# aquaskyline/SOAPdenovo-Trans

Hardware: AMD Instinct MI355X
Metric: pregraph k-mers hashed/sec (higher is better)
Workload: dtype u64

## Files before the change

soapdenovo-trans_amd/__init__.py:

```python
from __future__ import annotations

import ctypes
import os
import subprocess

import numpy as np

PKG_DIR = os.path.dirname(os.path.abspath(__file__))
CSRC_DIR = os.path.join(PKG_DIR, "csrc")
LIB_PATH = os.path.join(CSRC_DIR, "libsdt_gpu.so")
REPO_ROOT = os.path.dirname(PKG_DIR)

SDT_FLAG_DIRECT, SDT_FLAG_PARTITION, SDT_FLAG_TRACK_FIRST, SDT_FLAG_KEEP_READS, SDT_FLAG_CONTIG_INDEX = 1, 2, 4, 8, 16
SDT_OK, SDT_EINVAL, SDT_ENODEV, SDT_ENOMEM, SDT_EHIP, SDT_EFULL, SDT_ESTATE, SDT_ELIMIT = 0, -1, -2, -3, -4, -5, -6, -7

_c = ctypes
_ABI = [
    ("sdt_gpu_init", _c.c_int, [_c.POINTER(_c.c_void_p), _c.c_int, _c.c_int, _c.c_uint64, _c.c_uint32]),
    ("sdt_gpu_destroy", _c.c_int, [_c.c_void_p]),
    ("sdt_gpu_last_error", _c.c_char_p, []),
    ("sdt_gpu_abi_version", _c.c_int, []),
    ("sdt_gpu_reset", _c.c_int, [_c.c_void_p]),
    ("sdt_gpu_push_reads", _c.c_int, [_c.c_void_p, _c.c_void_p, _c.c_uint64, _c.c_void_p, _c.c_uint64]),
    ("sdt_gpu_push_reads_async", _c.c_int, [_c.c_void_p, _c.c_void_p, _c.c_uint64, _c.c_void_p, _c.c_uint64, _c.POINTER(_c.c_uint64)]),
# ... 888 lines not shown
        return fr[: n.value], to[: n.value], mult[: n.value], first[: n.value]

    def export_paths(self):
        n = ctypes.c_uint64()
        self._check(self.lib.sdt_gpu_export_paths(self._ctx, None, None, 0, ctypes.byref(n)))
        m = max(n.value, 1)
        keys = np.zeros((m, self.nw), dtype=np.uint64)
        words = np.zeros(m, dtype=np.uint64)
        self._check(self.lib.sdt_gpu_export_paths(self._ctx, _ptr(keys), _ptr(words), m, ctypes.byref(n)))
        return keys[: n.value], words[: n.value]

    def import_paths(self, keys, path_words, patch_keys=None, patch_info=None, num_ed: int = 0):
        keys = np.ascontiguousarray(keys, dtype=np.uint64).reshape(-1, self.nw)
        path_words = np.ascontiguousarray(path_words, dtype=np.uint64)
        assert len(keys) == len(path_words)
        pk, pi, npatch = self._patch_args(patch_keys, patch_info)
        self._check(self.lib.sdt_gpu_import_paths(self._ctx, _ptr(keys), _ptr(path_words), len(path_words), _ptr(pk), _ptr(pi), npatch,
                                                  num_ed))

    def keep_reads(self, words: np.ndarray, offsets: np.ndarray):
        words = np.ascontiguousarray(words, dtype=np.uint32)
        offsets = np.ascontiguousarray(offsets, dtype=np.uint64)
        self._check(self.lib.sdt_gpu_keep_reads(self._ctx, _ptr(words), words.size, _ptr(offsets), offsets.size - 1))

    def release_table(self):
        self._check(self.lib.sdt_gpu_release_table(self._ctx))

    def table_slots(self) -> int:
        return self.lib.sdt_gpu_table_slots(self._ctx)

    def table_info(self) -> dict:
        a = np.zeros(8, dtype=np.uint64)
        self._check(self.lib.sdt_gpu_table_info(self._ctx, a.ctypes.data))
        return {"layout": "flat", "slots": int(a[1]), "nodes": int(a[2])}

    def stream(self) -> int:
        return self.lib.sdt_gpu_stream(self._ctx) or 0

    def set_stream(self, hip_stream: int):
        self._check(self.lib.sdt_gpu_set_stream(self._ctx, ctypes.c_void_p(hip_stream)))

    def kernel_time(self, reset: bool = True):
        ms, launches, kmers = ctypes.c_double(), ctypes.c_uint64(), ctypes.c_uint64()
        self._check(self.lib.sdt_gpu_kernel_time(self._ctx, int(reset), ctypes.byref(ms), ctypes.byref(launches),
                                                 ctypes.byref(kmers)))
        return ms.value, launches.value, kmers.value

    def stage_times(self):
        ms = (ctypes.c_double * 5)()
        cnt = (ctypes.c_uint64 * 20)()
        self._check(self.lib.sdt_gpu_stage_times(self._ctx, ms, cnt))
        names = ("merges", "lds_spills", "pool_direct", "early_flushes", "chunks_l1", "chunks_l2", "batches", "batch_kmers", "cnt_ticks_setup",
                 "cnt_ticks_fill", "cnt_ticks_count", "cnt_ticks_merge", "sc_ticks_stage", "sc_ticks_minima", "sc_ticks_starts",
                 "sc_ticks_emit", "distinct_records", "records", "distinct_record_kmers", "reserved1")
        return [float(x) for x in ms], dict(zip(names, (int(x) for x in cnt)))


def new_comm_id() -> bytes:
    buf = ctypes.create_string_buffer(128)
    if load_library().sdt_gpu_comm_id(buf) != SDT_OK:
        raise SdtError(SDT_EHIP, load_library().sdt_gpu_last_error().decode())
    return buf.raw


def count_plan(off2, kpre2, first_limit, limit, max_launches=4096):
    o = np.ascontiguousarray(off2, dtype=np.uint32)
    kp = np.ascontiguousarray(kpre2, dtype=np.uint64)
    nb = len(o) - 1
    assert len(kp) == nb + 1
    cap = nb + int(o[-1]) // 1024 + 2
    items = np.zeros((cap, 4), dtype=np.uint32)
    first = np.zeros(max_launches + 2, dtype=np.uint32)
    lk = np.zeros(max_launches + 2, dtype=np.uint64)
    ni, nl = ctypes.c_uint32(), ctypes.c_uint32()
    rc = load_library().sdt_sk_plan_count_items(o.ctypes.data, kp.ctypes.data, nb, first_limit, limit, max_launches, items.ctypes.data, cap,
                                                first.ctypes.data, lk.ctypes.data, len(first), ctypes.addressof(ni), ctypes.addressof(nl))
    if rc != 0:
        raise SdtError(rc, load_library().sdt_gpu_last_error().decode())
    return items[: ni.value].copy(), first[: nl.value + 1].copy(), lk[: nl.value].copy()


def shard_cut_ranges(mat: np.ndarray, nranks: int) -> np.ndarray:
    m = np.ascontiguousarray(mat, dtype=np.uint32).reshape(nranks, 257)
    r = np.zeros(nranks + 1, dtype=np.uint32)
    rc = load_library().sdt_shard_cut_ranges(m.ctypes.data, nranks, r.ctypes.data)
    if rc != SDT_OK:
        raise SdtError(rc, load_library().sdt_gpu_last_error().decode())
    return r


def shard_plan(mat: np.ndarray, nranks: int, me: int, ranges: np.ndarray, recv_chunks: int, t: int):
    m = np.ascontiguousarray(mat, dtype=np.uint32).reshape(nranks, 257)
    rg = np.ascontiguousarray(ranges, dtype=np.uint32)
    S = ctypes.c_uint32()
    out = [np.zeros(nranks, dtype=np.uint32) for _ in range(5)]
    rc = load_library().sdt_shard_plan(m.ctypes.data, nranks, me, rg.ctypes.data, recv_chunks, t, ctypes.addressof(S),
                                       *[o.ctypes.data for o in out])
    if rc != SDT_OK:
        raise SdtError(rc, load_library().sdt_gpu_last_error().decode())
    return (S.value, *out)


def kmer_owner(key_words_msw_first, K: int, nranks: int) -> int:
    a = np.ascontiguousarray(key_words_msw_first, dtype=np.uint64)
    return load_library().sdt_kmer_owner(a.ctypes.data, K, nranks)


# ... 19 lines not shown
```

soapdenovo-trans_amd/csrc/sdt_ctx.hpp:

```cpp
#pragma once
#include <hip/hip_runtime.h>
#include <stdint.h>
#include <stdio.h>
#include <stdlib.h>
#include <string.h>
#include <stdarg.h>
#include <vector>
#include <new>
#include <thread>
#include <mutex>
#include <atomic>

#include "sdt_internal.hpp"
#include "sdt_superkmer.cuh"

using namespace sdt;
using sdti::fail;
#include "sdt_comm.cuh"
#include "sdt_shard_plan.h"
static_assert(SHARD_NB1 == SK_NB1, "the exchange plan and the pipeline agree about the level-1 buckets");

struct ArcEnt;

struct EventPair {
	hipEvent_t a, b;
	uint64_t kmers;
	int stage;
};

struct sdt_ctx {
	int device = 0;
	int K = 0;
	int nw = 1;
	uint64_t slots = 0;
	void *d_ent = nullptr;
	uint32_t *d_aux = nullptr;
	uint64_t *d_first = nullptr;
	uint64_t ord_base = 0, ord_stride = 1;
	Stats *d_stats = nullptr;
	Stats *h_stats = nullptr;
	unsigned long long *d_hist = nullptr;
	hipStream_t stream = nullptr, copy_stream = nullptr;
	bool own_stream = true;
	static constexpr int NSTAGE = 48, STAGE_AHEAD = 32;
	uint32_t *d_words[NSTAGE] = {};
	uint64_t *d_offs[NSTAGE] = {};
	uint64_t cap_words[NSTAGE] = {}, cap_offs[NSTAGE] = {};
	hipEvent_t buf_free[NSTAGE] = {}, copied[NSTAGE] = {};
	int next_buf = 0;
	struct Staged { const uint32_t *dw; uint64_t *dof; uint64_t nreads, maxlen, ord_base, ord_stride; int slot; uint64_t fixed_len; };
	std::vector<Staged> staged;
	size_t staged_head = 0;
	bool draining = false;
	uint64_t push_ord_base = 0, push_ord_stride = 1;
	uint64_t push_ticket = 0;
	uint64_t expect_kmers = 0;
	uint64_t distinct_known = 0;
	uint64_t kmers_known = 0;
	uint64_t kmers_since_sync = 0;
	uint64_t hard_since_sync = 0;
	uint64_t kmers_total_host = 0;
	uint64_t kmers_offered = 0;
	uint32_t flags = 0;
	struct SkState {
		bool ready = false;
		uint64_t cap_kmers = 0;
		bool cap_is_max = false;
		uint64_t pending_kmers = 0;
		SkPool p1 = {nullptr, nullptr, nullptr, 0}, p2 = {nullptr, nullptr, nullptr, 0};
		unsigned long long *cursors = nullptr;
		unsigned long long *blk = nullptr;
		uint32_t wgs = 0;
		uint32_t *cnt1 = nullptr, *off1 = nullptr, *fill1 = nullptr, *list1 = nullptr;
		uint32_t *cnt2 = nullptr, *off2 = nullptr, *fill2 = nullptr, *list2 = nullptr;
		unsigned long long *kmers2 = nullptr, *kpre2 = nullptr;
		SkItem *items = nullptr;
		uint32_t items_cap = 0;
		uint4 *citems = nullptr, *h_citems = nullptr;
		uint32_t citems_cap = 0;
		uint32_t *next_item = nullptr;
		uint32_t *h_off1 = nullptr, *h_off2 = nullptr;
		unsigned long long *h_kpre2 = nullptr;
		SkItem *h_items = nullptr;
		bool flushing = false;
		uint64_t st_records = 0, st_chunks1 = 0, st_chunks2 = 0, st_flushes = 0;
		uint32_t stream_flushes = 0;
		uint64_t l2_in_total = 0;
		bool exchanged = false;
	} sk;
	Comm comm;
	struct Shard {
		uint64_t *send[2] = {nullptr, nullptr}, *recv[2] = {nullptr, nullptr};
		uint32_t *send_meta[2] = {nullptr, nullptr}, *recv_meta[2] = {nullptr, nullptr};
		uint32_t *iota = nullptr;
		uint32_t send_chunks = 0, recv_chunks = 0;
		hipEvent_t ev_gather[2] = {nullptr, nullptr}, ev_xdone[2] = {nullptr, nullptr}, ev_l2[2] = {nullptr, nullptr};
		bool x_recorded[2] = {false, false}, l2_recorded[2] = {false, false};
		uint64_t round = 0;
		bool pending = false;
		int pending_slot = 0;
		uint32_t pending_items = 0;
		std::vector<SkItem> items;
		uint64_t kmers_scattered = 0;
		bool have_ranges = false;
		uint32_t ranges[65] = {0};
	} sh;
	struct KeptBatch { uint32_t *d_words; uint64_t *d_offs; uint64_t nwords, nreads, ord_base, ord_stride, maxlen; };
	std::vector<KeptBatch> kept;
	struct KeepSlab { uint8_t *p; size_t size, used; };
	std::vector<KeepSlab> keep_slabs;
	void *d_patch = nullptr;
	uint64_t patch_slots = 0;
	ArcEnt *d_arcs = nullptr;
	uint64_t arc_slots = 0;
	bool paths_loaded = false;
	uint64_t *d_idx = nullptr;
	sdti::GraphExt *gx = nullptr;
	uint64_t idx_slots = 0, idx_n = 0;
	uint32_t *d_ctg_ids = nullptr;
	uint64_t ctg_ord = 0, ctg_ids_cap = 0;
	uint32_t *d_ctg_len = nullptr, *d_ctg_twin = nullptr;
	uint64_t num_ctg = 0;
	void *ab[5] = {nullptr, nullptr, nullptr, nullptr, nullptr};
	size_t ab_cap[5] = {0, 0, 0, 0, 0};
	unsigned long long *d_hit_cursor = nullptr;
	bool index_final = false;
	uint64_t *d_hi = nullptr;
	uint64_t hi_slots = 0;
// ... 48 lines not shown
```

soapdenovo-trans_amd/csrc/sdt_gpu.hip:

```cpp
#include "sdt_ctx.hpp"
#include "sdt_pipeline.hpp"
#include "sdt_table_kernels.cuh"

static thread_local char g_err[512] = "";
static std::atomic<int> g_live_ctx{0};

int sdti::fail(int code, const char *fmt, ...)
{
	va_list ap;
	va_start(ap, fmt);
	vsnprintf(g_err, sizeof g_err, fmt, ap);
	va_end(ap);
	return code;
}
uint64_t flat_slots_for(uint64_t nodes)
{
	static const int pct = sdt_tuning_env("SDT_TABLE_LOAD") && atoi(sdt_tuning_env("SDT_TABLE_LOAD")) >= 10 && atoi(sdt_tuning_env("SDT_TABLE_LOAD")) <= 69 ? atoi(sdt_tuning_env("SDT_TABLE_LOAD")) : 45;
	uint64_t slots = (uint64_t)((double)nodes * 100.0 / pct) + 4095;
	slots &= ~4095ULL;
	return slots < (1ULL << 16) ? (1ULL << 16) : slots;
}

void *keep_alloc(sdt_ctx *c, size_t bytes)
{
// ... 858 lines not shown
	HIPCHK(hipMalloc((void **)&d_l, m * 4));
	HIPCHK(hipMalloc((void **)&d_r, m * 4));
	HIPCHK(hipMalloc((void **)&d_c, m * 4));
	if (first && c->d_first) HIPCHK(hipMalloc((void **)&d_f, m * 8));
	for (uint64_t i0 = 0; i0 < n && rc == SDT_OK; i0 += STEP) {
		const uint64_t k = n - i0 < STEP ? n - i0 : STEP;
		HIPCHK(hipMemcpyAsync(d_k, keys + i0 * c->nw, k * c->nw * 8, hipMemcpyHostToDevice, c->stream));
		HIPCHK(hipMemcpyAsync(d_l, l_links + i0, k * 4, hipMemcpyHostToDevice, c->stream));
		HIPCHK(hipMemcpyAsync(d_r, r_flags + i0, k * 4, hipMemcpyHostToDevice, c->stream));
		HIPCHK(hipMemcpyAsync(d_c, count + i0, k * 4, hipMemcpyHostToDevice, c->stream));
		if (d_f) HIPCHK(hipMemcpyAsync(d_f, first + i0, k * 8, hipMemcpyHostToDevice, c->stream));
		const int g = scan_grid(c, k);
		if (c->nw == 1) hipLaunchKernelGGL(k_import<1>, dim3(g), dim3(TPB), 0, c->stream, flat_of<1>(c), d_k, d_l, d_r, d_c, d_f, k, c->d_stats);
		else if (c->nw == 2) hipLaunchKernelGGL(k_import<2>, dim3(g), dim3(TPB), 0, c->stream, flat_of<2>(c), d_k, d_l, d_r, d_c, d_f, k, c->d_stats);
		else hipLaunchKernelGGL(k_import<4>, dim3(g), dim3(TPB), 0, c->stream, flat_of<4>(c), d_k, d_l, d_r, d_c, d_f, k, c->d_stats);
		HIPCHK(hipGetLastError());
		HIPCHK(hipStreamSynchronize(c->stream));
	}
	(void)hipFree(d_k); (void)hipFree(d_l); (void)hipFree(d_r); (void)hipFree(d_c);
	if (d_f) (void)hipFree(d_f);
	return sync_stats(c);
}
int sdt_gpu_stage_times(sdt_ctx *c, double ms[SDT_NSTAGES], uint64_t counters[SDT_NCOUNTERS])
{
	if (!c)
		return fail(SDT_EINVAL, "ctx is NULL");
	HIPCHK(hipSetDevice(c->device));
	HIPCHK(hipStreamSynchronize(c->stream));
	if (ms) {
		for (int i = 0; i < SDT_NSTAGES; i++) ms[i] = 0;
		for (size_t i = 0; i < c->ev_used; i++) {
			float t = 0;
			HIPCHK(hipEventElapsedTime(&t, c->ev[i].a, c->ev[i].b));
			ms[c->ev[i].stage] += t;
		}
	}
	if (counters) {
		HIPCHK(hipMemcpy(c->h_stats, c->d_stats, sizeof(Stats), hipMemcpyDeviceToHost));
		counters[0] = c->h_stats->sk_merges;
		counters[1] = c->h_stats->sk_spills;
		counters[2] = c->h_stats->sk_direct;
		counters[3] = c->h_stats->sk_gens;
		counters[4] = c->sk.st_chunks1;
		counters[5] = c->sk.st_chunks2;
		counters[6] = c->sk.st_flushes;
		counters[7] = c->sk.cap_kmers;
		for (int i = 0; i < 4; i++)
			counters[8 + i] = c->h_stats->sk_cyc[i];
		for (int i = 0; i < 4; i++)
			counters[12 + i] = c->h_stats->sk_cyc1[i];
		counters[16] = c->h_stats->sk_distinct_recs;
		counters[17] = c->h_stats->sk_records;
		counters[18] = c->h_stats->sk_distinct_kmers;
		counters[19] = 0;
	}
	return SDT_OK;
}
}

int drain_pushes(sdt_ctx *c, bool force) { return drain_staged(c, force); }

sdti::GraphView sdti::graph_view(sdt_ctx *c)
{
	GraphView v;
	v.device = c->device; v.K = c->K; v.nw = c->nw; v.cu_count = c->cu_count;
	v.slots = view_slots(c);
	v.d_ent = c->d_ent; v.d_aux = c->d_aux; v.d_first = c->d_first;
	v.d_stats = c->d_stats; v.h_stats = c->h_stats;
	v.stream = c->stream; v.copy_stream = c->copy_stream;
	v.d_idx = &c->d_idx; v.idx_slots = &c->idx_slots; v.idx_n = &c->idx_n;
	v.gx = &c->gx;
	return v;
}

int sdti::sync_stats(sdt_ctx *c) { return ::sync_stats(c); }

int sdti::drop_first(sdt_ctx *c)
{
	HIPCHK(hipSetDevice(c->device));
	if (c->d_first) { HIPCHK(hipFree(c->d_first)); c->d_first = nullptr; }
	return SDT_OK;
}

int sdti::release_pass1(sdt_ctx *c)
{
	const int rc = ::sync_stats(c);
	if (rc != SDT_OK) return rc;
	if (!sdt_tuning_env("SDT_KEEP_POOLS")) {
		sk_free(c);
	}
	return SDT_OK;
}
struct BigStage {
	static constexpr int NB = 4;
	static constexpr size_t CH = (size_t)32 << 20;
	void *pin[NB] = {};
	hipEvent_t done[NB] = {};
	bool ok = false;
	std::mutex mu;
	bool init()
	{
		if (ok) return true;
		for (int i = 0; i < NB; i++)
			if (hipHostMalloc(&pin[i], CH, hipHostMallocDefault) != hipSuccess || hipEventCreateWithFlags(&done[i], hipEventDisableTiming) != hipSuccess)
				return false;
		ok = true;
		return true;
// ... 67 lines not shown
```

soapdenovo-trans_amd/csrc/sdt_pipeline.hip:

```cpp
#include "sdt_ctx.hpp"
#include "sdt_tile.cuh"
#include "sdt_superkmer_kernels.cuh"
#include "sdt_count_plan.h"
#include "sdt_pipeline.hpp"

void sk_free(sdt_ctx *c)
{
	sdt_ctx::SkState &k = c->sk;
	void *dev[] = {k.p1.recs, k.p1.meta, k.p1.next, k.p2.recs, k.p2.meta, k.p2.next, k.cursors, k.blk, k.cnt1, k.off1, k.fill1, k.list1,
	               k.cnt2, k.off2, k.fill2, k.list2, k.kmers2, k.kpre2, k.items, k.citems, k.next_item};
	for (void *p : dev)
		if (p) (void)hipFree(p);
	void *host[] = {k.h_off1, k.h_off2, k.h_kpre2, k.h_items, k.h_citems};
	for (void *p : host)
		if (p) (void)hipHostFree(p);
	const uint64_t in_total = k.l2_in_total;
	const bool exchanged = k.exchanged;
	const uint32_t stream_flushes = k.stream_flushes;
	k = sdt_ctx::SkState();
	k.l2_in_total = in_total;
	k.exchanged = exchanged;
	k.stream_flushes = stream_flushes;
}

SkGeo sk_geo(int K, uint64_t max_read_len)
{
	SkGeo g;
	g.mtw = (int)(((uint64_t)SK_TILE_READS * max_read_len + 16 + 15) / 16) + TAIL_PAD + 1;
	g.tile_words = (int)((tile_smem_bytes(g.mtw) / sizeof(uint32_t) + 1) & ~(size_t)1);
	g.hv_words = (int)((SK_TILE_READS * max_read_len + 16 + 1) & ~(uint64_t)1);
	const uint64_t nk_max = (uint64_t)SK_TILE_READS * (max_read_len - K + 1);
	g.bits_words = (int)(nk_max / 64 + 2);
	g.hv2_words = K - sk_minimizer_len(K) + 1 > 49 ? g.hv_words : 0;
	g.smem = (size_t)g.tile_words * 4 + (size_t)SK_NB1 * 8 + (size_t)(g.hv_words + g.hv2_words) * 4 + (size_t)g.bits_words * 8 + (size_t)(g.bits_words + 2) * 4;
	return g;
}

template <int NW, bool TRACK> static size_t sk_count_smem()
{
	using G = SkCntGeo<NW, TRACK>;
	constexpr int SLOTS = G::SLOTS, BW = SkFmt<NW>::BW, TR = G::TILE;
	return (size_t)(NW + (TRACK ? 1 : 0)) * SLOTS * 8 + (size_t)TR * 8 + (size_t)SLOTS * 20 + (size_t)TR * 4 + G::REGION +
	       (size_t)(LDS_LEAD + TR * BW * 2 + TAIL_PAD) * 4;
}

bool sk_applicable(const sdt_ctx *c, uint64_t max_read_len)
{
	if (c->flags & SDT_FLAG_CONTIG_INDEX)
		return false;
	if (max_read_len < (uint64_t)c->K + 1 || max_read_len > (uint64_t)SK_MAX_READ_LEN)
		return false;
	return sk_geo(c->K, max_read_len).smem <= 160 * 1024;
}

int sk_reset_pool1(sdt_ctx *c)
{
	sdt_ctx::SkState &k = c->sk;
	HIPCHK(hipMemsetAsync(k.p1.next, 0, 4, c->stream));
	HIPCHK(hipMemsetAsync(k.cnt1, 0, SK_NB1 * 4, c->stream));
	hipLaunchKernelGGL(k_sk_init_cursors, dim3(256), dim3(256), 0, c->stream, k.cursors, k.wgs * (uint32_t)SK_NB1, (uint32_t)SK_CAP1, k.blk, k.wgs);
	HIPCHK(hipGetLastError());
	k.pending_kmers = 0;
	return SDT_OK;
// ... 13 lines not shown
	const int rw = sk_rec_words(c->nw), rw2 = sk_rec2_stride(c->nw);
	const int w = c->K - sk_minimizer_len(c->K) + 1;
	const double rate = 2.0 / (double)(w + 1) + 1.0 / (double)sk_max_run(c->K, c->nw);
	double run = 1.0 / rate * ((c->nw == 4 || per_read > (uint64_t)SK_SEQ_MAX_KMERS) ? 0.8 : 1.0);
	if (run > (double)per_read) run = (double)per_read;
	uint64_t div = (uint64_t)run;
	if (div < 2) div = 2;
	div = (uint64_t)clamp_int(sdt_knob_int(sdt_tuning_env("SDT_SK_POOL_DIV"), (int)div), 1, 1 << 20);
	const int mem_pct = sdt_knob_int(sdt_tuning_env("SDT_SK_POOL_MEM_PCT"), 70);
	size_t free_b = 0, total_b = 0;
	HIPCHK(sdti::mem_info(&free_b, &total_b));
	uint64_t cap = want_kmers < (1ULL << 24) ? (1ULL << 24) : want_kmers;
	k.cap_is_max = cap >= SK_BATCH_MAX_KMERS;
	const uint32_t wgs = (uint32_t)c->cu_count * 6;
	for (;; cap /= 2) {
		const uint64_t recs = cap / div;
		const uint64_t chunks1 = sdt_knob_int(sdt_test_env("SDT_SK_POOL_CHUNKS1"), 0) > 0 ? (uint64_t)sdt_knob_int(sdt_test_env("SDT_SK_POOL_CHUNKS1"), 0) : recs / SK_CAP1 + (uint64_t)wgs * SK_NB1 + 1024;
		const uint64_t items = chunks1 / SK_ITEM_CHUNKS + SK_NB1 + 1;
		const uint64_t chunks2 = chunks1 * (SK_CAP1 / SK_CAP2) + items * (SK_NB2 + SK_BLK2) + 1024;
		const uint64_t bytes = chunks1 * SK_CAP1 * rw * 8 + chunks2 * SK_CAP2 * rw2 * 8 + (chunks1 + chunks2) * 8;
		const uint64_t all = c->comm.nranks > 1 ? bytes + chunks1 * SK_CAP1 * rw * 8 * 9 / 2 : bytes;
		if (chunks2 >= (1ULL << SK_LIST2_FILL_SHIFT) - 1 || all > free_b / 100 * (uint64_t)mem_pct) {
			k.cap_is_max = true;
			if (cap <= (1ULL << 24))
				return fail(SDT_ENOMEM, "super-k-mer pools: %llu MiB needed for the smallest batch, %zu MiB free",
				            (unsigned long long)(bytes >> 20), free_b >> 20);
			continue;
		}
		k.p1.chunks = (uint32_t)chunks1;
		k.p2.chunks = (uint32_t)chunks2;
		k.items_cap = (uint32_t)items;
		break;
	}
	k.wgs = wgs;
	const double t_alloc0 = comm_now();
	HIPCHK(hipMalloc((void **)&k.p1.recs, (size_t)k.p1.chunks * SK_CAP1 * rw * 8));
	HIPCHK(hipMalloc((void **)&k.p1.meta, (size_t)k.p1.chunks * 4));
	HIPCHK(hipMalloc((void **)&k.p1.next, 64));
	HIPCHK(hipMalloc((void **)&k.p2.recs, (size_t)k.p2.chunks * SK_CAP2 * rw2 * 8));
	HIPCHK(hipMalloc((void **)&k.p2.meta, (size_t)k.p2.chunks * 4));
	HIPCHK(hipMalloc((void **)&k.p2.next, 64));
	HIPCHK(hipMalloc((void **)&k.cursors, (size_t)wgs * SK_NB1 * 8));
	HIPCHK(hipMalloc((void **)&k.blk, (size_t)wgs * 8));
	HIPCHK(hipMalloc((void **)&k.cnt1, SK_NB1 * 4));
	HIPCHK(hipMalloc((void **)&k.off1, (SK_NB1 + 1) * 4));
	HIPCHK(hipMalloc((void **)&k.fill1, SK_NB1 * 4));
	HIPCHK(hipMalloc((void **)&k.list1, (size_t)k.p1.chunks * 4));
	HIPCHK(hipMalloc((void **)&k.cnt2, SK_NBF * 4));
	HIPCHK(hipMalloc((void **)&k.off2, (SK_NBF + 1) * 4));
	HIPCHK(hipMalloc((void **)&k.fill2, SK_NBF * 4));
	HIPCHK(hipMalloc((void **)&k.list2, (size_t)k.p2.chunks * 4));
	HIPCHK(hipMalloc((void **)&k.kmers2, SK_NBF * 8));
	HIPCHK(hipMalloc((void **)&k.kpre2, (SK_NBF + 1) * 8));
	HIPCHK(hipMalloc((void **)&k.items, (size_t)k.items_cap * sizeof(SkItem)));
	HIPCHK(hipHostMalloc((void **)&k.h_off1, (SK_NB1 + 1) * 4, hipHostMallocDefault));
	HIPCHK(hipHostMalloc((void **)&k.h_off2, (SK_NBF + 1) * 4, hipHostMallocDefault));
	HIPCHK(hipHostMalloc((void **)&k.h_kpre2, (SK_NBF + 1) * 8, hipHostMallocDefault));
	HIPCHK(hipHostMalloc((void **)&k.h_items, (size_t)k.items_cap * sizeof(SkItem), hipHostMallocDefault));
	k.citems_cap = (uint32_t)SK_NBF + k.p2.chunks / SK_COUNT_ITEM_CHUNKS + 1;
	HIPCHK(hipMalloc((void **)&k.citems, (size_t)k.citems_cap * sizeof(uint4)));
	HIPCHK(hipHostMalloc((void **)&k.h_citems, (size_t)k.citems_cap * sizeof(uint4), hipHostMallocDefault));
	HIPCHK(hipMalloc((void **)&k.next_item, SK_MAX_COUNT_LAUNCHES * sizeof(uint32_t)));
	k.cap_kmers = cap;
	k.ready = true;
	if (sdt_env("SDT_TIMING"))
		fprintf(stderr, "[libsdt_gpu] super-k-mer pools for %llu k-mers per batch: %.1f GiB in %.0f ms\n", (unsigned long long)cap,
		        ((double)k.p1.chunks * SK_CAP1 * rw + (double)k.p2.chunks * SK_CAP2 * rw2) * 8 / (1 << 30), (comm_now() - t_alloc0) * 1e3);
	return sk_reset_pool1(c);
}

template <int NW, bool TRACK> static int sk_launch_count_t(sdt_ctx *c, uint32_t i0, uint32_t i1, uint32_t launch)
{
	sdt_ctx::SkState &k = c->sk;
	const size_t smem = sk_count_smem<NW, TRACK>();
	const unsigned per_cu = (unsigned)((160 * 1024) / (smem + 256));
	unsigned grid = (unsigned)c->cu_count * (per_cu < 1 ? 1 : (per_cu > 2 ? 2 : per_cu));
	if (grid > i1 - i0) grid = i1 - i0;
	HIPCHK(hipFuncSetAttribute((const void *)k_sk_count<NW, TRACK>, hipFuncAttributeMaxDynamicSharedMemorySize, (int)smem));
	hipLaunchKernelGGL((k_sk_count<NW, TRACK>), dim3(grid), dim3(SkCntGeo<NW, TRACK>::TPB), smem, c->stream, k.p2, k.list2, (const uint4 *)k.citems, i0, i1,
	                   k.next_item + launch, c->K, flat_of<NW>(c), c->d_stats);
	HIPCHK(hipGetLastError());
	return SDT_OK;
}

template <int NW> static int sk_launch_count(sdt_ctx *c, uint32_t i0, uint32_t i1, uint32_t launch)
{
	return c->d_first ? sk_launch_count_t<NW, true>(c, i0, i1, launch) : sk_launch_count_t<NW, false>(c, i0, i1, launch);
}


int sk_list1(sdt_ctx *c)
{
	sdt_ctx::SkState &k = c->sk;
	const int g = c->cu_count * 8;
	hipLaunchKernelGGL(k_sk_seal, dim3(256), dim3(256), 0, c->stream, k.cursors, k.wgs * (uint32_t)SK_NB1, k.blk, k.wgs, k.p1, (uint32_t)SK_CAP1);
	hipLaunchKernelGGL(k_sk_scan, dim3(1), dim3(1024), 0, c->stream, k.cnt1, k.off1, k.fill1, (int)SK_NB1, (const unsigned long long *)nullptr, (unsigned long long *)nullptr);
	hipLaunchKernelGGL(k_sk_chunk_place_few, dim3(g), dim3(256), 0, c->stream, k.p1, k.off1, k.fill1, k.list1, (int)SK_NB1);
	SK_CHK(hipGetLastError());
	SK_CHK(hipMemcpyAsync(k.h_off1, k.off1, (SK_NB1 + 1) * 4, hipMemcpyDeviceToHost, c->stream));
	{ const int rcw = c->comm.sync_watched(c->stream, "the chunk lists of a round"); if (rcw != SDT_OK) return rcw; }
	k.st_chunks1 = k.h_off1[SK_NB1];
	return SDT_OK;
}

int sk_split(sdt_ctx *c, const SkPool &src, const uint32_t *list, uint32_t nitems, hipEvent_t after_l2)
{
	sdt_ctx::SkState &k = c->sk;
	const int g = c->cu_count * 8;
	SK_CHK(hipMemsetAsync(k.p2.next, 0, 4, c->stream));
	SK_CHK(hipMemsetAsync(k.kmers2, 0, SK_NBF * 8, c->stream));
	SK_CHK(hipMemsetAsync(k.cnt2, 0, SK_NBF * 4, c->stream));
	if (nitems) {
		SK_CHK(hipMemcpyAsync(k.items, k.h_items, (size_t)nitems * sizeof(SkItem), hipMemcpyHostToDevice, c->stream));
		const size_t sm = c->nw == 1 ? SkL2Stage<1>::SMEM : (c->nw == 2 ? SkL2Stage<2>::SMEM : SkL2Stage<4>::SMEM);
		const void *fn = c->nw == 1 ? (const void *)k_sk_scatter_records_staged<1> : (c->nw == 2 ? (const void *)k_sk_scatter_records_staged<2> : (const void *)k_sk_scatter_records_staged<4>);
		SK_CHK(hipFuncSetAttribute(fn, hipFuncAttributeMaxDynamicSharedMemorySize, (int)sm));
		if (c->nw == 1) hipLaunchKernelGGL(k_sk_scatter_records_staged<1>, dim3(nitems), dim3(SK_L2S_TPB), sm, c->stream, src, list, k.items, k.p2, k.cnt2, k.kmers2, c->d_stats);
		else if (c->nw == 2) hipLaunchKernelGGL(k_sk_scatter_records_staged<2>, dim3(nitems), dim3(SK_L2S_TPB), sm, c->stream, src, list, k.items, k.p2, k.cnt2, k.kmers2, c->d_stats);
		else hipLaunchKernelGGL(k_sk_scatter_records_staged<4>, dim3(nitems), dim3(SK_L2S_TPB), sm, c->stream, src, list, k.items, k.p2, k.cnt2, k.kmers2, c->d_stats);
		SK_CHK(hipGetLastError());
	}
	if (after_l2)
		SK_CHK(hipEventRecord(after_l2, c->stream));
	hipLaunchKernelGGL(k_sk_scan, dim3(1), dim3(1024), 0, c->stream, k.cnt2, k.off2, k.fill2, (int)SK_NBF, (const unsigned long long *)k.kmers2, k.kpre2);
	hipLaunchKernelGGL(k_sk_chunk_place, dim3(g), dim3(256), 0, c->stream, k.p2, k.off2, k.fill2, k.list2);
	SK_CHK(hipGetLastError());
	SK_CHK(hipMemcpyAsync(k.h_kpre2, k.kpre2, (SK_NBF + 1) * 8, hipMemcpyDeviceToHost, c->stream));
	SK_CHK(hipMemcpyAsync(k.h_off2, k.off2, (SK_NBF + 1) * 4, hipMemcpyDeviceToHost, c->stream));
	return SDT_OK;
}

int sk_count_all(sdt_ctx *c)
{
	sdt_ctx::SkState &k = c->sk;
	SK_CHK(hipStreamSynchronize(c->stream));
	k.st_chunks2 = k.h_off2[SK_NBF];
	k.st_flushes++;
	k.stream_flushes++;
	k.l2_in_total += k.h_kpre2[SK_NBF];
	int rc = SDT_OK;
	uint32_t nci = 0;
	SK_CHK(hipMemsetAsync(k.next_item, 0, SK_MAX_COUNT_LAUNCHES * sizeof(uint32_t), c->stream));
	std::vector<uint32_t> first_item(SK_MAX_COUNT_LAUNCHES + 2);
	std::vector<uint64_t> launch_kmers(SK_MAX_COUNT_LAUNCHES + 2);
	uint32_t nlaunches = 0;
	
	if (!sk_plan_count_items(k.h_off2, (const uint64_t *)k.h_kpre2, (uint32_t)SK_NBF, c->kmers_known == 0 ? (1ULL << 26) : SK_COUNT_KMERS, SK_COUNT_KMERS,
	                         SK_MAX_COUNT_LAUNCHES, SK_COUNT_PACK_CHUNKS, SK_COUNT_ITEM_CHUNKS, (uint32_t *)k.h_citems, k.citems_cap,
	                         first_item.data(), launch_kmers.data(), (uint32_t)first_item.size(), &nci, &nlaunches))
		return fail(SDT_ESTATE, "count stage: work item table overflow");
	first_item.resize(nlaunches + 1);
	launch_kmers.resize(nlaunches);
	std::vector<uint32_t> sort_tmp;
	auto guess_of = [&](uint64_t kmers) -> uint64_t {
		uint64_t bound = kmers;
		if (c->kmers_known) {
			const double rate = (double)c->distinct_known / (double)c->kmers_known;
			const uint64_t guess = (uint64_t)((double)kmers * (2.0 * rate < 1.0 ? 2.0 * rate : 1.0)) + (1ULL << 22);
			if (guess < bound) bound = guess;
		}
		return bound;
	};
	const size_t nl = first_item.size() - 1;
	for (size_t l = 0; l < nl && rc == SDT_OK;) {
		const uint32_t i0 = first_item[l];
		if (i0 == first_item[l + 1]) {
			l++;
			continue;
		}
		if (c->kmers_known == 0 && l > 0) {
			rc = sync_stats(c);
			if (rc != SDT_OK) break;
		}
		uint64_t bound = guess_of(launch_kmers[l]), hard = launch_kmers[l];
		rc = ensure_room(c, bound);
		if (rc == SDT_OK && (double)(c->distinct_known + c->hard_since_sync + launch_kmers[l]) > 0.95 * (double)c->slots) {
			rc = sync_stats(c);
// ... 230 lines not shown
```

soapdenovo-trans_amd/csrc/sdt_superkmer_kernels.cuh:

```cuda
#pragma once

#ifndef SDT_SK_PREFETCH
#define SDT_SK_PREFETCH 1
#endif
#ifndef SDT_SK_CLAIM_BELOW
#define SDT_SK_CLAIM_BELOW 0
#endif
#ifndef SDT_SK_LOAD16
#define SDT_SK_LOAD16 1
#endif
#ifndef SDT_SK_CLAIM2_BELOW
#define SDT_SK_CLAIM2_BELOW 0
#endif
#ifndef SDT_SK_FLUSH_NUM
#define SDT_SK_FLUSH_NUM 4
#endif
#ifndef SDT_SK_NW2_TWO
#define SDT_SK_NW2_TWO 1
#endif
#ifndef SDT_SK_SEQ_FLUSH
#define SDT_SK_SEQ_FLUSH 1
#endif
#ifndef SDT_SK_CNT_TPB
#define SDT_SK_CNT_TPB 1024
// ... 230 lines not shown
				}
			}
		}
		__syncthreads();
		SK_TICK(3);
	}
#undef SK_TICK
	for (int i = tid; i < SK_NB1; i += TPB) {
		g_cursors[(size_t)blockIdx.x * SK_NB1 + i] = s_cur[i];
		if (s_cnt[i])
			atomicAdd(&g_cnt[i], s_cnt[i]);
	}
	if (tid == 0) {
		g_blk[blockIdx.x] = s_blk;
#ifdef SDT_SK_TICKS
		for (int i = 0; i < 4; i++)
			atomicAdd(&stats->sk_cyc1[i], cyc[i]);
#endif
	}
	if (done) {
		atomicAdd(&stats->kmers, (unsigned long long)done);
		atomicAdd(&stats->sk_direct, (unsigned long long)done);
	}
	if (claimed) atomicAdd(&stats->distinct, (unsigned long long)claimed);
	if (failed) atomicAdd(&stats->probe_fail, (unsigned long long)failed);
#pragma unroll
	for (int d = 32; d > 0; d >>= 1)
		emitted += __shfl_down(emitted, d);
	if ((tid & 63) == 0 && emitted)
		atomicAdd(&stats->sk_emitted, (unsigned long long)emitted);
}

static __global__ __launch_bounds__(256) void k_sk_seal(const unsigned long long *__restrict__ cursors, uint32_t n, const unsigned long long *__restrict__ blk,
                                                 uint32_t nblk, SkPool pool, uint32_t cap)
{
	for (uint32_t i = blockIdx.x * 256u + threadIdx.x; i < n; i += gridDim.x * 256u) {
		const unsigned long long cur = cursors[i];
		const uint32_t chunk = (uint32_t)(cur >> 32), pos = (uint32_t)cur;
		if (chunk != SK_NOCHUNK)
			pool.meta[chunk] = (pool.meta[chunk] & 0xFFFFFFu) | ((pos < cap ? pos : cap) << 24);
	}
	for (uint32_t i = blockIdx.x * 256u + threadIdx.x; i < nblk; i += gridDim.x * 256u)
		sk_retire_block(blk[i], pool);
}

static __global__ __launch_bounds__(256) void k_sk_init_cursors(unsigned long long *cursors, uint32_t n, uint32_t cap, unsigned long long *blk, uint32_t nblk)
{
	for (uint32_t i = blockIdx.x * 256u + threadIdx.x; i < n; i += gridDim.x * 256u)
		cursors[i] = ((unsigned long long)SK_NOCHUNK << 32) | cap;
	for (uint32_t i = blockIdx.x * 256u + threadIdx.x; i < nblk; i += gridDim.x * 256u)
		blk[i] = 0;
}

static __global__ __launch_bounds__(1024) void k_sk_scan(const uint32_t *__restrict__ cnt, uint32_t *__restrict__ off, uint32_t *__restrict__ fillcur,
                                                  int nb, const unsigned long long *__restrict__ kmers, unsigned long long *__restrict__ kpre)
{
	__shared__ unsigned long long s_a[1024], s_b[1024];
	const int t = threadIdx.x, per = (nb + 1023) / 1024;
	const int i0 = t * per, i1 = i0 + per < nb ? i0 + per : nb;
	unsigned long long a = 0, b = 0;
	for (int i = i0; i < i1; i++) {
		a += cnt[i];
		if (kmers) b += kmers[i];
	}
	s_a[t] = a;
	s_b[t] = b;
	__syncthreads();
	for (int d = 1; d < 1024; d <<= 1) {
		const unsigned long long va = t >= d ? s_a[t - d] : 0, vb = t >= d ? s_b[t - d] : 0;
		__syncthreads();
		s_a[t] += va;
		s_b[t] += vb;
		__syncthreads();
	}
	a = t ? s_a[t - 1] : 0;
	b = t ? s_b[t - 1] : 0;
	for (int i = i0; i < i1; i++) {
		off[i] = (uint32_t)a;
		fillcur[i] = 0;
		a += cnt[i];
		if (kmers) {
			kpre[i] = b;
			b += kmers[i];
		}
	}
	if (t == 1023) {
		off[nb] = (uint32_t)s_a[1023];
		if (kmers) kpre[nb] = s_b[1023];
	}
}

static __global__ __launch_bounds__(256) void k_sk_chunk_place(SkPool pool, const uint32_t *__restrict__ off, uint32_t *__restrict__ fillcur,
                                                        uint32_t *__restrict__ list)
{
	const uint32_t used = *pool.next, n = used < pool.chunks ? used : pool.chunks;
	for (uint32_t c = blockIdx.x * 256u + threadIdx.x; c < n; c += gridDim.x * 256u) {
		const uint32_t mt = pool.meta[c];
		if (mt == SK_DEAD)
			continue;
		const uint32_t b = mt & 0xFFFFFFu;
		list[off[b] + atomicAdd(&fillcur[b], 1u)] = c | (((mt >> 24) - 1u) << SK_LIST2_FILL_SHIFT);
	}
}

static __global__ __launch_bounds__(256) void k_sk_chunk_place_few(SkPool pool, const uint32_t *__restrict__ off, uint32_t *__restrict__ fillcur,
                                                            uint32_t *__restrict__ list, int nb)
{
	__shared__ uint32_t s_cnt[1024], s_base[1024];
	constexpr uint32_t STRETCH = 256u * 16u;
	const uint32_t used = *pool.next, n = used < pool.chunks ? used : pool.chunks;
	for (uint32_t c0 = blockIdx.x * STRETCH; c0 < n; c0 += gridDim.x * STRETCH) {
		for (int i = threadIdx.x; i < nb; i += 256)
			s_cnt[i] = 0;
		__syncthreads();
		uint32_t mine[16], bucket[16];
#pragma unroll
		for (int t = 0; t < 16; t++) {
			const uint32_t c = c0 + (uint32_t)t * 256u + threadIdx.x;
			const uint32_t mt = c < n ? pool.meta[c] : SK_DEAD;
			bucket[t] = mt == SK_DEAD ? 0xFFFFFFFFu : (mt & 0xFFFFFFu);
			mine[t] = mt == SK_DEAD ? 0u : atomicAdd(&s_cnt[bucket[t]], 1u);
		}
		__syncthreads();
		for (int i = threadIdx.x; i < nb; i += 256)
			s_base[i] = s_cnt[i] ? atomicAdd(&fillcur[i], s_cnt[i]) : 0u;
		__syncthreads();
#pragma unroll
		for (int t = 0; t < 16; t++)
			if (bucket[t] != 0xFFFFFFFFu)
				list[off[bucket[t]] + s_base[bucket[t]] + mine[t]] = c0 + (uint32_t)t * 256u + threadIdx.x;
		__syncthreads();
	}
}


#ifdef SDT_SK_L2_LOG
__device__ unsigned long long *g_l2_log = nullptr;
__device__ unsigned long long g_l2_log_cap = 0;
#endif

#ifndef SDT_SK_L2S_S1
#define SDT_SK_L2S_S1 4
#endif
#ifndef SDT_SK_L2S_WGS
#define SDT_SK_L2S_WGS 1
#endif
#ifndef SDT_SK_L2S_RPL
#define SDT_SK_L2S_RPL 2
#endif
template <int NW> struct SkL2Stage {
	static constexpr int S = NW == 1 ? SDT_SK_L2S_S1 : 2;
	static constexpr int GPC = SK_CAP2 / S;
	static constexpr int RPL = NW == 1 ? SDT_SK_L2S_RPL : (NW == 2 ? (SDT_SK_L2S_RPL < 2 ? SDT_SK_L2S_RPL : 2) : 1);
	static constexpr size_t SMEM = (size_t)SK_NB2 * S * SkFmt<NW>::REC_WORDS * 8;
};

template <int NW>
__global__ __launch_bounds__(SK_L2S_TPB, SDT_SK_L2S_WGS) void k_sk_scatter_records_staged(SkPool src, const uint32_t *__restrict__ list1,
                                                                         const SkItem *__restrict__ items, SkPool dst,
                                                                         uint32_t *__restrict__ g_cnt, unsigned long long *__restrict__ g_kmers, Stats *stats)
{
	constexpr int RW = SkFmt<NW>::REC_WORDS, RW2 = SkFmt<NW>::REC2_STRIDE, S = SkL2Stage<NW>::S, GPC = SkL2Stage<NW>::GPC;
	constexpr int CPT = SK_L2S_TPB / SK_CAP1;
	constexpr int D = SkL2Stage<NW>::RPL;
	extern __shared__ unsigned long long s_stage[];
	__shared__ uint32_t s_cnt[SK_NB2];
	__shared__ uint32_t s_open[SK_NB2];
	__shared__ uint32_t s_pub_open[SK_NB2], s_pub_new[SK_NB2], s_pub_g[SK_NB2];
	__shared__ unsigned char s_fill[SK_NB2], s_used[SK_NB2];
	__shared__ uint32_t s_kc[SK_NB2], s_cc[SK_NB2];
	__shared__ unsigned long long s_blk;
	const SkItem it = items[blockIdx.x];
	const int tid = threadIdx.x;
	for (int i = tid; i < SK_NB2; i += SK_L2S_TPB) {
		s_cnt[i] = 0;
		s_open[i] = SK_NOCHUNK;
		s_fill[i] = 0;
		s_used[i] = 0;
		s_kc[i] = 0;
		s_cc[i] = 0;
	}
	if (tid == 0)
		s_blk = 0;
	__syncthreads();
	uint32_t failed = 0;
	auto alloc = [&](uint32_t n) -> uint32_t {
		const uint32_t id = sk_alloc_chunks(&s_blk, dst, n, SK_BLK2);
		return id < dst.chunks && id + n <= dst.chunks ? id : SK_NOCHUNK;
	};
	auto slot_of = [&](uint32_t open, uint32_t used, uint32_t first_new, uint32_t t) -> uint64_t * {
		const uint32_t a = (open == SK_NOCHUNK ? (uint32_t)GPC : used) + t / S;
		if (a < (uint32_t)GPC)
			return dst.recs + ((size_t)open * SK_CAP2 + a * S + t % S) * RW2;
		if (first_new == SK_NOCHUNK)
			return nullptr;
		return dst.recs + ((size_t)(first_new + (a - GPC) / GPC) * SK_CAP2 + ((a - GPC) % GPC) * S + t % S) * RW2;
	};
	const uint32_t slot = (uint32_t)tid % SK_CAP1, cfirst = it.c0 + (uint32_t)tid / SK_CAP1;
	uint32_t id_a[D], id_b[D], fill_a[D];
	uint64_t rec_a[D][RW];
#pragma unroll
	for (int d = 0; d < D; d++) {
		const uint32_t ca = cfirst + (uint32_t)d * CPT, cb = ca + (uint32_t)D * CPT;
		id_a[d] = ca < it.c1 ? list1[ca] : SK_NOCHUNK;
		id_b[d] = cb < it.c1 ? list1[cb] : SK_NOCHUNK;
	}
#pragma unroll
	for (int d = 0; d < D; d++) {
		fill_a[d] = 0;
#pragma unroll
		for (int i = 0; i < RW; i++)
			rec_a[d][i] = 0;
		if (id_a[d] != SK_NOCHUNK) {
			fill_a[d] = src.meta[id_a[d]] >> 24;
			sk_load_record<RW>(src.recs + ((size_t)id_a[d] * SK_CAP1 + slot) * RW, rec_a[d]);
		}
	}
	const uint32_t nsweep = (it.c1 - it.c0 + CPT - 1) / CPT;
	for (uint32_t sw = 0; sw < nsweep; sw += (uint32_t)D) {
		uint64_t rec[D][RW];
		uint32_t b2[D], t[D];
		bool valid[D];
#pragma unroll
		for (int d = 0; d < D; d++) {
			const uint32_t ci = cfirst + (sw + (uint32_t)d) * CPT;
#pragma unroll
			for (int i = 0; i < RW; i++)
				rec[d][i] = rec_a[d][i];
			const uint32_t fill = ci < it.c1 ? fill_a[d] : 0u;
			id_a[d] = id_b[d];
			const uint32_t cn = ci + 2u * (uint32_t)D * CPT;
			id_b[d] = cn < it.c1 ? list1[cn] : SK_NOCHUNK;
			if (id_a[d] != SK_NOCHUNK) {
				fill_a[d] = src.meta[id_a[d]] >> 24;
				sk_load_record<RW>(src.recs + ((size_t)id_a[d] * SK_CAP1 + slot) * RW, rec_a[d]);
			}
			valid[d] = slot < fill;
			b2[d] = 0;
			t[d] = 0;
			if (valid[d]) {
				b2[d] = sk_hdr_l2(rec[d][0]);
				t[d] = atomicAdd(&s_cnt[b2[d]], 1u);
				atomicAdd(&s_kc[b2[d]], (uint32_t)sk_hdr_n(rec[d][0]));
			}
		}
		__syncthreads();
		for (int i = tid; i < SK_NB2; i += SK_L2S_TPB) {
			const uint32_t f = s_fill[i], total = s_cnt[i];
			if (total == f)
				continue;
			const uint32_t G = total / S, left = total - G * S;
			const uint32_t open = s_open[i], used = open == SK_NOCHUNK ? (uint32_t)GPC : s_used[i];
			const uint32_t room = (uint32_t)GPC - used;
			uint32_t first_new = SK_NOCHUNK;
			if (G > room) {
				const uint32_t nnew = (G - room + GPC - 1) / GPC;
				first_new = alloc(nnew);
				if (first_new != SK_NOCHUNK) {
					for (uint32_t j = 0; j < nnew; j++)
						dst.meta[first_new + j] = (it.b1 * SK_NB2 + (uint32_t)i) | ((uint32_t)SK_CAP2 << 24);
					s_cc[i] += nnew;
				}
			}
			s_pub_open[i] = open;
			s_pub_new[i] = first_new;
			s_pub_g[i] = used | (G << 8);
			if (G && f) {
				for (uint32_t j = 0; j < f; j++) {
					uint64_t old[RW];
#pragma unroll
					for (int w = 0; w < RW; w++)
						old[w] = s_stage[((size_t)i * S + j) * RW + w];
					uint64_t *p = slot_of(open, used, first_new, j);
					if (p) sk_store_record2<NW>(p, old);
					else failed++;
				}
			}
			if (G) {
				const uint32_t a_end = used + G;
				if (a_end <= (uint32_t)GPC) {
					s_used[i] = (unsigned char)a_end;
				} else if (first_new != SK_NOCHUNK) {
					s_open[i] = first_new + (a_end - GPC - 1) / GPC;
					s_used[i] = (unsigned char)((a_end - GPC - 1) % GPC + 1);
				} else {
					s_open[i] = SK_NOCHUNK;
					s_used[i] = 0;
				}
			}
			s_fill[i] = (unsigned char)left;
			s_cnt[i] = left;
		}
		__syncthreads();
#pragma unroll
		for (int d = 0; d < D; d++) {
			if (!valid[d])
				continue;
			const uint32_t g = s_pub_g[b2[d]], G = g >> 8, used = g & 0xFFu;
			if (t[d] / S < G) {
				uint64_t *p = slot_of(s_pub_open[b2[d]], used, s_pub_new[b2[d]], t[d]);
				if (p) sk_store_record2<NW>(p, rec[d]);
				else failed++;
			} else {
				const uint32_t at = t[d] - G * S;
#pragma unroll
				for (int i = 0; i < RW; i++)
					s_stage[((size_t)b2[d] * S + at) * RW + i] = rec[d][i];
			}
		}
	}
	__syncthreads();
	for (int i = tid; i < SK_NB2; i += SK_L2S_TPB) {
		const uint32_t f = s_fill[i];
		uint32_t open = s_open[i], used = open == SK_NOCHUNK ? (uint32_t)GPC : s_used[i];
		if (f) {
			if (used == (uint32_t)GPC) {
				open = alloc(1);
				used = 0;
				if (open != SK_NOCHUNK)
					s_cc[i]++;
			}
			if (open != SK_NOCHUNK) {
				for (uint32_t j = 0; j < f; j++) {
					uint64_t rec[RW];
#pragma unroll
					for (int w = 0; w < RW; w++)
						rec[w] = s_stage[((size_t)i * S + j) * RW + w];
					sk_store_record2<NW>(dst.recs + ((size_t)open * SK_CAP2 + used * S + j) * RW2, rec);
				}
			} else {
				failed += f;
			}
		}
		if (open != SK_NOCHUNK)
			dst.meta[open] = (it.b1 * SK_NB2 + (uint32_t)i) | ((used * S + f) << 24);
		if (s_kc[i])
			atomicAdd(&g_kmers[it.b1 * SK_NB2 + i], (unsigned long long)s_kc[i]);
		if (s_cc[i])
			atomicAdd(&g_cnt[it.b1 * SK_NB2 + i], s_cc[i]);
	}
	__syncthreads();
	{
		const unsigned long long blk = s_blk;
		const uint32_t next = (uint32_t)blk, end = (uint32_t)(blk >> 32);
		for (uint32_t id = next + (uint32_t)tid; id < end && id < dst.chunks; id += SK_L2S_TPB)
			dst.meta[id] = SK_DEAD;
	}
	if (failed)
		atomicAdd(&stats->probe_fail, (unsigned long long)failed);
}

struct SkGatherPlan {
	uint32_t begin[64];
	uint32_t pre[65];
	uint32_t dst0[64];
	int n, self;
};

template <int RW>
__global__ __launch_bounds__(256) void k_sk_gather(SkPool pool, const uint32_t *__restrict__ list, SkGatherPlan plan,
                                                   uint64_t *__restrict__ send, uint32_t *__restrict__ send_meta,
                                                   uint64_t *__restrict__ recv, uint32_t *__restrict__ recv_meta)
{
// ... 554 lines not shown
```

Measured before the change: 95.05 billion.

## Pipeline L2 scatter loads/stores across rounds and parallelize the bucket scan

The level-2 scatter loop now issues the next round's chunk-list, meta and record loads before processing the current round. It also defers each round's global and LDS stores into the following iteration, with a scheduling barrier, so memory latency overlaps the atomic counting and publication phases. Out-of-range chunk ids are clamped to a valid index instead of skipped, which adds some redundant loads. The single-workgroup prefix scan over level-2 buckets is replaced by a two-kernel tiled scan across many workgroups, and a probe_fail counter is exposed in the stats.

```diff
diff --git a/soapdenovo-trans_amd/__init__.py b/soapdenovo-trans_amd/__init__.py
--- a/soapdenovo-trans_amd/__init__.py
+++ b/soapdenovo-trans_amd/__init__.py
@@ -964,7 +964,7 @@
         self._check(self.lib.sdt_gpu_stage_times(self._ctx, ms, cnt))
         names = ("merges", "lds_spills", "pool_direct", "early_flushes", "chunks_l1", "chunks_l2", "batches", "batch_kmers", "cnt_ticks_setup",
                  "cnt_ticks_fill", "cnt_ticks_count", "cnt_ticks_merge", "sc_ticks_stage", "sc_ticks_minima", "sc_ticks_starts",
-                 "sc_ticks_emit", "distinct_records", "records", "distinct_record_kmers", "reserved1")
+                 "sc_ticks_emit", "distinct_records", "records", "distinct_record_kmers", "probe_fail")
         return [float(x) for x in ms], dict(zip(names, (int(x) for x in cnt)))
 
 
diff --git a/soapdenovo-trans_amd/csrc/sdt_ctx.hpp b/soapdenovo-trans_amd/csrc/sdt_ctx.hpp
--- a/soapdenovo-trans_amd/csrc/sdt_ctx.hpp
+++ b/soapdenovo-trans_amd/csrc/sdt_ctx.hpp
@@ -74,6 +74,7 @@
 		uint32_t *cnt1 = nullptr, *off1 = nullptr, *fill1 = nullptr, *list1 = nullptr;
 		uint32_t *cnt2 = nullptr, *off2 = nullptr, *fill2 = nullptr, *list2 = nullptr;
 		unsigned long long *kmers2 = nullptr, *kpre2 = nullptr;
+		unsigned long long *scan2 = nullptr;
 		SkItem *items = nullptr;
 		uint32_t items_cap = 0;
 		uint4 *citems = nullptr, *h_citems = nullptr;
diff --git a/soapdenovo-trans_amd/csrc/sdt_gpu.hip b/soapdenovo-trans_amd/csrc/sdt_gpu.hip
--- a/soapdenovo-trans_amd/csrc/sdt_gpu.hip
+++ b/soapdenovo-trans_amd/csrc/sdt_gpu.hip
@@ -934,7 +934,7 @@
 		counters[16] = c->h_stats->sk_distinct_recs;
 		counters[17] = c->h_stats->sk_records;
 		counters[18] = c->h_stats->sk_distinct_kmers;
-		counters[19] = 0;
+		counters[19] = c->h_stats->probe_fail;
 	}
 	return SDT_OK;
 }
diff --git a/soapdenovo-trans_amd/csrc/sdt_pipeline.hip b/soapdenovo-trans_amd/csrc/sdt_pipeline.hip
--- a/soapdenovo-trans_amd/csrc/sdt_pipeline.hip
+++ b/soapdenovo-trans_amd/csrc/sdt_pipeline.hip
@@ -8,7 +8,7 @@
 {
 	sdt_ctx::SkState &k = c->sk;
 	void *dev[] = {k.p1.recs, k.p1.meta, k.p1.next, k.p2.recs, k.p2.meta, k.p2.next, k.cursors, k.blk, k.cnt1, k.off1, k.fill1, k.list1,
-	               k.cnt2, k.off2, k.fill2, k.list2, k.kmers2, k.kpre2, k.items, k.citems, k.next_item};
+	               k.cnt2, k.off2, k.fill2, k.list2, k.kmers2, k.kpre2, k.scan2, k.items, k.citems, k.next_item};
 	for (void *p : dev)
 		if (p) (void)hipFree(p);
 	void *host[] = {k.h_off1, k.h_off2, k.h_kpre2, k.h_items, k.h_citems};
@@ -128,6 +128,7 @@
 	HIPCHK(hipMalloc((void **)&k.list2, (size_t)k.p2.chunks * 4));
 	HIPCHK(hipMalloc((void **)&k.kmers2, SK_NBF * 8));
 	HIPCHK(hipMalloc((void **)&k.kpre2, (SK_NBF + 1) * 8));
+	HIPCHK(hipMalloc((void **)&k.scan2, (size_t)((SK_NBF + SK_SCAN_TILE - 1) / SK_SCAN_TILE) * 2 * 8));
 	HIPCHK(hipMalloc((void **)&k.items, (size_t)k.items_cap * sizeof(SkItem)));
 	HIPCHK(hipHostMalloc((void **)&k.h_off1, (SK_NB1 + 1) * 4, hipHostMallocDefault));
 	HIPCHK(hipHostMalloc((void **)&k.h_off2, (SK_NBF + 1) * 4, hipHostMallocDefault));
@@ -198,7 +199,10 @@
 	}
 	if (after_l2)
 		SK_CHK(hipEventRecord(after_l2, c->stream));
-	hipLaunchKernelGGL(k_sk_scan, dim3(1), dim3(1024), 0, c->stream, k.cnt2, k.off2, k.fill2, (int)SK_NBF, (const unsigned long long *)k.kmers2, k.kpre2);
+	const unsigned scan_tiles = (unsigned)((SK_NBF + SK_SCAN_TILE - 1) / SK_SCAN_TILE);
+	hipLaunchKernelGGL(k_sk_scan_sums, dim3(scan_tiles), dim3(SK_SCAN_TILE), 0, c->stream, k.cnt2, (const unsigned long long *)k.kmers2, (int)SK_NBF, k.scan2);
+	hipLaunchKernelGGL(k_sk_scan_tiles, dim3(scan_tiles), dim3(SK_SCAN_TILE), 0, c->stream, k.cnt2, k.off2, k.fill2, (int)SK_NBF, (const unsigned long long *)k.kmers2, k.kpre2,
+	                   (const unsigned long long *)k.scan2);
 	hipLaunchKernelGGL(k_sk_chunk_place, dim3(g), dim3(256), 0, c->stream, k.p2, k.off2, k.fill2, k.list2);
 	SK_CHK(hipGetLastError());
 	SK_CHK(hipMemcpyAsync(k.h_kpre2, k.kpre2, (SK_NBF + 1) * 8, hipMemcpyDeviceToHost, c->stream));
diff --git a/soapdenovo-trans_amd/csrc/sdt_superkmer_kernels.cuh b/soapdenovo-trans_amd/csrc/sdt_superkmer_kernels.cuh
--- a/soapdenovo-trans_amd/csrc/sdt_superkmer_kernels.cuh
+++ b/soapdenovo-trans_amd/csrc/sdt_superkmer_kernels.cuh
@@ -306,6 +306,21 @@
 		blk[i] = 0;
 }
 
+__device__ inline void sk_scan_1024(unsigned long long a, unsigned long long b, unsigned long long *s_a, unsigned long long *s_b)
+{
+	const int t = threadIdx.x;
+	s_a[t] = a;
+	s_b[t] = b;
+	__syncthreads();
+	for (int d = 1; d < 1024; d <<= 1) {
+		const unsigned long long va = t >= d ? s_a[t - d] : 0, vb = t >= d ? s_b[t - d] : 0;
+		__syncthreads();
+		s_a[t] += va;
+		s_b[t] += vb;
+		__syncthreads();
+	}
+}
+
 static __global__ __launch_bounds__(1024) void k_sk_scan(const uint32_t *__restrict__ cnt, uint32_t *__restrict__ off, uint32_t *__restrict__ fillcur,
                                                   int nb, const unsigned long long *__restrict__ kmers, unsigned long long *__restrict__ kpre)
 {
@@ -317,16 +332,7 @@
 		a += cnt[i];
 		if (kmers) b += kmers[i];
 	}
-	s_a[t] = a;
-	s_b[t] = b;
-	__syncthreads();
-	for (int d = 1; d < 1024; d <<= 1) {
-		const unsigned long long va = t >= d ? s_a[t - d] : 0, vb = t >= d ? s_b[t - d] : 0;
-		__syncthreads();
-		s_a[t] += va;
-		s_b[t] += vb;
-		__syncthreads();
-	}
+	sk_scan_1024(a, b, s_a, s_b);
 	a = t ? s_a[t - 1] : 0;
 	b = t ? s_b[t - 1] : 0;
 	for (int i = i0; i < i1; i++) {
@@ -344,6 +350,43 @@
 	}
 }
 
+constexpr int SK_SCAN_TILE = 1024;
+static_assert(SK_NBF <= SK_SCAN_TILE * SK_SCAN_TILE, "one lane per tile adds up the tiles before a tile");
+static __global__ __launch_bounds__(SK_SCAN_TILE) void k_sk_scan_sums(const uint32_t *__restrict__ cnt, const unsigned long long *__restrict__ kmers, int nb,
+                                                                     unsigned long long *__restrict__ sums)
+{
+	__shared__ unsigned long long s_a[SK_SCAN_TILE], s_b[SK_SCAN_TILE];
+	const int i = (int)blockIdx.x * SK_SCAN_TILE + (int)threadIdx.x;
+	sk_scan_1024(i < nb ? cnt[i] : 0, i < nb ? kmers[i] : 0, s_a, s_b);
+	if (threadIdx.x == 0) {
+		sums[2 * blockIdx.x] = s_a[SK_SCAN_TILE - 1];
+		sums[2 * blockIdx.x + 1] = s_b[SK_SCAN_TILE - 1];
+	}
+}
+
+static __global__ __launch_bounds__(SK_SCAN_TILE) void k_sk_scan_tiles(const uint32_t *__restrict__ cnt, uint32_t *__restrict__ off, uint32_t *__restrict__ fillcur,
+                                                                      int nb, const unsigned long long *__restrict__ kmers, unsigned long long *__restrict__ kpre,
+                                                                      const unsigned long long *__restrict__ sums)
+{
+	__shared__ unsigned long long s_a[SK_SCAN_TILE], s_b[SK_SCAN_TILE];
+	const int t = threadIdx.x, i = (int)blockIdx.x * SK_SCAN_TILE + t;
+	const bool before = t < (int)blockIdx.x;
+	sk_scan_1024(before ? sums[2 * t] : 0, before ? sums[2 * t + 1] : 0, s_a, s_b);
+	const unsigned long long base_a = s_a[SK_SCAN_TILE - 1], base_b = s_b[SK_SCAN_TILE - 1];
+	__syncthreads();
+	const unsigned long long a = i < nb ? cnt[i] : 0, b = i < nb ? kmers[i] : 0;
+	sk_scan_1024(a, b, s_a, s_b);
+	if (i < nb) {
+		off[i] = (uint32_t)(base_a + s_a[t] - a);
+		fillcur[i] = 0;
+		kpre[i] = base_b + s_b[t] - b;
+		if (i == nb - 1) {
+			off[nb] = (uint32_t)(base_a + s_a[t]);
+			kpre[nb] = base_b + s_b[t];
+		}
+	}
+}
+
 static __global__ __launch_bounds__(256) void k_sk_chunk_place(SkPool pool, const uint32_t *__restrict__ off, uint32_t *__restrict__ fillcur,
                                                         uint32_t *__restrict__ list)
 {
@@ -398,6 +441,9 @@
 #endif
 #ifndef SDT_SK_L2S_WGS
 #define SDT_SK_L2S_WGS 1
+#endif
+#ifndef SDT_SK_L2S_ROTATE
+#define SDT_SK_L2S_ROTATE 1
 #endif
 #ifndef SDT_SK_L2S_RPL
 #define SDT_SK_L2S_RPL 2
@@ -451,44 +497,80 @@
 		return dst.recs + ((size_t)(first_new + (a - GPC) / GPC) * SK_CAP2 + ((a - GPC) % GPC) * S + t % S) * RW2;
 	};
 	const uint32_t slot = (uint32_t)tid % SK_CAP1, cfirst = it.c0 + (uint32_t)tid / SK_CAP1;
-	uint32_t id_a[D], id_b[D], fill_a[D];
-	uint64_t rec_a[D][RW];
+	uint32_t ld_id[D], ld_meta[D];
+	uint64_t ld_rec[D][RW];
+	auto list_at = [&](uint32_t c) -> uint32_t { return list1[c < it.c1 ? c : it.c0]; };
+	auto ask = [&](int d, uint32_t id) {
+		ld_meta[d] = src.meta[id];
+		sk_load_record<RW>(src.recs + ((size_t)id * SK_CAP1 + slot) * RW, ld_rec[d]);
+	};
 #pragma unroll
 	for (int d = 0; d < D; d++) {
-		const uint32_t ca = cfirst + (uint32_t)d * CPT, cb = ca + (uint32_t)D * CPT;
-		id_a[d] = ca < it.c1 ? list1[ca] : SK_NOCHUNK;
-		id_b[d] = cb < it.c1 ? list1[cb] : SK_NOCHUNK;
-	}
+		const uint32_t ca = cfirst + (uint32_t)d * CPT;
+		const uint32_t id0 = list_at(ca);
+		ld_id[d] = list_at(ca + (uint32_t)D * CPT);
+		ask(d, id0);
+	}
+	auto store_round = [&](const uint64_t (&rec)[D][RW], const uint32_t (&b2)[D], const uint32_t (&t)[D], const bool (&valid)[D]) {
+#pragma unroll
+		for (int d = 0; d < D; d++) {
+			if (!valid[d])
+				continue;
+			const uint32_t g = s_pub_g[b2[d]], G = g >> 8, used = g & 0xFFu;
+			if (t[d] / S < G) {
+				uint64_t *p = slot_of(s_pub_open[b2[d]], used, s_pub_new[b2[d]], t[d]);
+				if (p) sk_store_record2<NW>(p, rec[d]);
+				else failed++;
+			} else {
+				const uint32_t at = t[d] - G * S;
+#pragma unroll
+				for (int i = 0; i < RW; i++)
+					s_stage[((size_t)b2[d] * S + at) * RW + i] = rec[d][i];
+			}
+		}
+	};
+#if SDT_SK_L2S_ROTATE
+	uint64_t prec[D][RW];
+	uint32_t pb2[D], pt[D];
+	bool pvalid[D];
 #pragma unroll
 	for (int d = 0; d < D; d++) {
-		fill_a[d] = 0;
+		pvalid[d] = false;
+		pb2[d] = pt[d] = 0;
 #pragma unroll
 		for (int i = 0; i < RW; i++)
-			rec_a[d][i] = 0;
-		if (id_a[d] != SK_NOCHUNK) {
-			fill_a[d] = src.meta[id_a[d]] >> 24;
-			sk_load_record<RW>(src.recs + ((size_t)id_a[d] * SK_CAP1 + slot) * RW, rec_a[d]);
-		}
-	}
+			prec[d][i] = 0;
+	}
+#endif
 	const uint32_t nsweep = (it.c1 - it.c0 + CPT - 1) / CPT;
 	for (uint32_t sw = 0; sw < nsweep; sw += (uint32_t)D) {
 		uint64_t rec[D][RW];
-		uint32_t b2[D], t[D];
+		uint32_t b2[D], t[D], meta[D], idn[D];
 		bool valid[D];
+#pragma unroll
+		for (int d = 0; d < D; d++) {
+			meta[d] = ld_meta[d];
+			idn[d] = ld_id[d];
+			asm volatile("" : "+v"(meta[d]), "+v"(idn[d]));
+#pragma unroll
+			for (int i = 0; i < RW; i++) {
+				rec[d][i] = ld_rec[d][i];
+				asm volatile("" : "+v"(rec[d][i]));
+			}
+		}
+#pragma unroll
+		for (int d = 0; d < D; d++) {
+			ld_id[d] = list_at(cfirst + (sw + (uint32_t)d + 2u * (uint32_t)D) * CPT);
+			ask(d, idn[d]);
+		}
+		__builtin_amdgcn_sched_barrier(0);
+#if SDT_SK_L2S_ROTATE
+		store_round(prec, pb2, pt, pvalid);
+#endif
 #pragma unroll
 		for (int d = 0; d < D; d++) {
 			const uint32_t ci = cfirst + (sw + (uint32_t)d) * CPT;
-#pragma unroll
-			for (int i = 0; i < RW; i++)
-				rec[d][i] = rec_a[d][i];
-			const uint32_t fill = ci < it.c1 ? fill_a[d] : 0u;
-			id_a[d] = id_b[d];
-			const uint32_t cn = ci + 2u * (uint32_t)D * CPT;
-			id_b[d] = cn < it.c1 ? list1[cn] : SK_NOCHUNK;
-			if (id_a[d] != SK_NOCHUNK) {
-				fill_a[d] = src.meta[id_a[d]] >> 24;
-				sk_load_record<RW>(src.recs + ((size_t)id_a[d] * SK_CAP1 + slot) * RW, rec_a[d]);
-			}
+			const uint32_t fill = ci < it.c1 ? meta[d] >> 24 : 0u;
 			valid[d] = slot < fill;
 			b2[d] = 0;
 			t[d] = 0;
@@ -546,23 +628,22 @@
 			s_cnt[i] = left;
 		}
 		__syncthreads();
+#if SDT_SK_L2S_ROTATE
 #pragma unroll
 		for (int d = 0; d < D; d++) {
-			if (!valid[d])
-				continue;
-			const uint32_t g = s_pub_g[b2[d]], G = g >> 8, used = g & 0xFFu;
-			if (t[d] / S < G) {
-				uint64_t *p = slot_of(s_pub_open[b2[d]], used, s_pub_new[b2[d]], t[d]);
-				if (p) sk_store_record2<NW>(p, rec[d]);
-				else failed++;
-			} else {
-				const uint32_t at = t[d] - G * S;
-#pragma unroll
-				for (int i = 0; i < RW; i++)
-					s_stage[((size_t)b2[d] * S + at) * RW + i] = rec[d][i];
-			}
-		}
-	}
+			pvalid[d] = valid[d];
+			pb2[d] = b2[d];
+			pt[d] = t[d];
+#pragma unroll
+			for (int i = 0; i < RW; i++)
+				prec[d][i] = rec[d][i];
+		}
+	}
+	store_round(prec, pb2, pt, pvalid);
+#else
+		store_round(rec, b2, t, valid);
+	}
+#endif
 	__syncthreads();
 	for (int i = tid; i < SK_NB2; i += SK_L2S_TPB) {
 		const uint32_t f = s_fill[i];
```

After: 92.44 billion. 0.973x the previous value.
